# nihalsid/retrieval-fuse

Hardware: AMD Instinct MI355X
Metric: 64^3 TSDF chunks/sec (retrieve+attend+refine) (higher is better)
Workload: dtype f32

## Files before the change

retrieval-fuse_amd/csrc/build.py:

```python
import os
import subprocess
import sys
from concurrent.futures import ThreadPoolExecutor
from pathlib import Path

HERE = Path(__file__).resolve().parent
OUT = HERE.parent / 'rfuse' / 'librfuse_hip.so'
SOURCES = ['capi.hip', 'conv3d.hip', 'conv3d_mfma.hip', 'conv3d_up.hip', 'conv3d_up_split.hip', 'conv3d_split.hip', 'conv3d_split_zc.hip', 'conv3d_e2_split.hip', 'conv3d_small.hip', 'conv3d_backward.hip', 'conv3d_wgrad_split.hip', 'conv_valid_mfma.hip', 'conv_valid_split.hip', 'conv_valid_split_pg.hip', 'conv_valid_backward.hip', 'linear.hip', 'attention.hip', 'attention_fused.hip', 'retrieval.hip', 'mesh.hip', 'metrics.hip', 'mesh_metrics.hip']
FLAGS = ['--offload-arch=gfx950', '-O3', '-std=c++17', '-fPIC', '-Wall', '-Wno-unused-function']
EXTRA_FLAGS = {'attention.hip': ['-ffp-contract=off'], 'attention_fused.hip': ['-ffp-contract=off'], 'retrieval.hip': ['-ffp-contract=off'],
               'mesh_metrics.hip': ['-ffp-contract=off'],
               'conv3d_mfma.hip': ['-fno-slp-vectorize'], 'conv3d_up.hip': ['-fno-slp-vectorize']}


def _hipcc():
    return os.environ.get('HIPCC', '/opt/rocm/bin/hipcc')


def _llvm_bin():
    import shutil
    roots = [Path(os.path.realpath(_hipcc())).parents[1], Path(os.environ.get('ROCM_PATH', '/opt/rocm')), Path('/opt/rocm')]
    for r in roots:
        for sub in ('lib/llvm/bin', 'llvm/bin'):
            if (r / sub / 'llvm-objdump').exists():
# ... 33 lines not shown
        for co in cos:
            asm = subprocess.run([str(llvm_bin / 'llvm-objdump'), '-d', str(co)], check=True, capture_output=True, text=True).stdout
            bad += unsafe_packed_fp32(asm)
    if bad:
        raise RuntimeError('check_isa: %d packed-fp32 instructions with op_sel on src1/src2 (wrong results beside F16 MFMAs on gfx950), e.g.\n  %s'
                           % (len(bad), '\n  '.join(bad[:5])))
    return len(cos)


def build(force=False, verbose=False, out=None, extra_flags=(), objdir=None):
    hipcc = _hipcc()
    OUT = Path(out) if out is not None else globals()['OUT']
    objdir = Path(objdir) if objdir is not None else HERE / 'build'
    objdir.mkdir(exist_ok=True, parents=True)
    headers = [HERE / 'common.h', HERE / 'conv_box.h', HERE / 'conv_split_common.h', HERE / 'split_operand.h', HERE / 'attn_row.h', HERE / 'philox.h',
               HERE.parents[1] / 'include' / 'rfuse.h', HERE.parents[1] / 'include' / 'rfuse_eval.h']

    def compile_one(src):
        obj = objdir / (src.replace('.hip', '.o'))
        if force or _stale(obj, [HERE / src, HERE / 'build.py'] + headers):
            cmd = [hipcc] + FLAGS + list(extra_flags) + EXTRA_FLAGS.get(src, []) + ['-c', str(HERE / src), '-o', str(obj)]
            if verbose:
                print(' '.join(cmd))
            subprocess.run(cmd, check=True)
        return obj

    with ThreadPoolExecutor(max_workers=len(SOURCES)) as ex:
        objs = list(ex.map(compile_one, SOURCES))
    if force or _stale(OUT, objs):
        tmp_out = OUT.with_name(OUT.name + '.unchecked')
        cmd = [hipcc, '--offload-arch=gfx950', '-shared', '-fPIC', '-o', str(tmp_out)] + [str(o) for o in objs]
# ... 27 lines not shown
```

retrieval-fuse_amd/csrc/conv3d_split.hip:

```cpp
#include "common.h"
#include "conv_box.h"
#include "conv_split_common.h"
#include <type_traits>

bool rf_split_zc_takes(int cin, int n, int edge, int cout);
int rf_split_zc_launch(const ConvArgs& a, const SplitPreOut& po, hipStream_t stream);
bool rf_split_zcm_takes(int cin, int n, int edge, int cout);
int rf_split_zcm_launch(const ConvArgs& a, const SplitPreOut& po, bool pre, hipStream_t stream, const char* who);
int rf_split_zcm_launch_ch8_pointwise(const ConvArgs& a, const SplitPreOut& po, hipStream_t stream, const char* who);

extern "C" size_t rf_conv3_split_packed_bytes(int cout, int cin) {
    return ((size_t)((cin + 7) / 8) * 7 + 1) * (size_t)(rf_round_up(cout, 16) / 16) * 2 * 64 * 16;
}

__global__ void k_conv3_split_pack(const float* __restrict__ w, int cout, int cin, int nb_count, h8* __restrict__ wp, size_t total) {
    const size_t nreal = (size_t)((cin + 7) / 8) * 7 * nb_count * 128;
    for (size_t i = (size_t)blockIdx.x * blockDim.x + threadIdx.x; i < total; i += (size_t)gridDim.x * blockDim.x) {
        const int lane = (int)(i & 63), piece = (int)((i >> 6) & 1);
        const size_t f = i >> 7;
        const int nb = (int)(f % nb_count);
        const size_t st = f / nb_count;
        const int co = nb * 16 + (lane & 15), g = lane >> 4;
        const int s = (int)(st % 7), ca = (int)(st / 7), tap = 4 * s + g;
        h8 out;
// ... 395 lines not shown
    conv_box_epilogue<4, 4, 4, 8, 8, 4, NB, (size_t)S4_LDS_BYTES>(a, acc, reinterpret_cast<float*>(lds), tid, lane, wave, n0, 0, 0, 0, cob, lblock);
}

struct Cin1PreArgs {
    const float* src;
    const float* gamma_in;
    const float* beta_in;
    double eps_in;
    const float* wp;
    int n, cin4, cout16;
    const float* gamma;
    const float* beta;
    int cpg;
    double eps;
    unsigned char* out;
};

__global__ __launch_bounds__(512, 4) void k_conv3_cin1_presplit(Cin1PreArgs a) {
    constexpr int E = 16, H = 18, VOL = E * E * E;
    __shared__ float xs[H * H * H];
    __shared__ __attribute__((aligned(16))) float wl[27 * 8];
    __shared__ double red[8 * 16];
    __shared__ float4 nxt[8];
    const int tid = threadIdx.x, lane = tid & 63, wave = tid >> 6;
    const int nn = blockIdx.x;
    for (int i = tid; i < H * H * H; i += 512) xs[i] = 0.f;
    for (int i = tid; i < 27 * 8; i += 512) wl[i] = a.wp[(size_t)(i / 8) * a.cin4 * a.cout16 + (i % 8)];
    const float* src = a.src + (size_t)nn * VOL;
    float raw[8];
#pragma unroll
    for (int i = 0; i < 8; ++i) raw[i] = src[tid + i * 512];
    {
        double sm = 0.0, sq = 0.0;
#pragma unroll
        for (int i = 0; i < 8; ++i) { sm += (double)raw[i]; sq += (double)raw[i] * raw[i]; }
        sm = wave_sum(sm); sq = wave_sum(sq);
        if (lane == 0) { red[2 * wave] = sm; red[2 * wave + 1] = sq; }
    }
    __syncthreads();
    float4 af;
    {
        double sm = 0.0, sq = 0.0;
        for (int w = 0; w < 8; ++w) { sm += red[2 * w]; sq += red[2 * w + 1]; }
        af = rf_gn_triple(sm, sq, VOL, a.eps_in, a.gamma_in[0], a.beta_in[0]);
    }
    __syncthreads();
#pragma unroll
    for (int i = 0; i < 8; ++i) {
        const int v = tid + i * 512;
        xs[((v >> 8) + 1) * (H * H) + (((v >> 4) & 15) + 1) * H + (v & 15) + 1] = fmaf(raw[i] - af.x, af.y, af.z);
    }
    __syncthreads();
    const int x = tid & 15, y = (tid >> 4) & 15, z0 = (tid >> 8) * 8;
    typedef float f32x2 __attribute__((ext_vector_type(2)));
    f32x2 acc2[8][4];
#pragma unroll
    for (int z = 0; z < 8; ++z)
#pragma unroll
        for (int cp = 0; cp < 4; ++cp) acc2[z][cp] = (f32x2){0.f, 0.f};
#pragma unroll
    for (int dy = 0; dy < 3; ++dy)
// ... 8 lines not shown
                const float4 w1 = *reinterpret_cast<const float4*>(wl + ((dz * 3 + dy) * 3 + dx) * 8 + 4);
                const f32x2 wv[4] = {(f32x2){w0.x, w0.y}, (f32x2){w0.z, w0.w}, (f32x2){w1.x, w1.y}, (f32x2){w1.z, w1.w}};
#pragma unroll
                for (int z = 0; z < 8; ++z) {
                    const f32x2 c2 = (f32x2){col[z + dz], col[z + dz]};
#pragma unroll
                    for (int cp = 0; cp < 4; ++cp) acc2[z][cp] = __builtin_elementwise_fma(c2, wv[cp], acc2[z][cp]);
                }
            }
        }
    float act[8][8];
#pragma unroll
    for (int z = 0; z < 8; ++z)
#pragma unroll
        for (int co = 0; co < 8; ++co) act[z][co] = rf_relu(acc2[z][co >> 1][co & 1]);
    {
        double v[16];
#pragma unroll
        for (int co = 0; co < 8; ++co) {
            double sm = 0.0, sq = 0.0;
#pragma unroll
            for (int z = 0; z < 8; ++z) { const double t = (double)act[z][co]; sm += t; sq += t * t; }
            v[2 * co] = sm; v[2 * co + 1] = sq;
        }
        auto halve = [&](auto kc) {
            constexpr int K = decltype(kc)::value, C = 8 >> K;
            const bool up = (lane >> K) & 1;
#pragma unroll
            for (int i = 0; i < C; ++i) {
                const double send = up ? v[i] : v[i + C], keep = up ? v[i + C] : v[i];
                v[i] = keep + __shfl_xor(send, 1 << K, 64);
            }
        };
        halve(std::integral_constant<int, 0>{});
        halve(std::integral_constant<int, 1>{});
        halve(std::integral_constant<int, 2>{});
        halve(std::integral_constant<int, 3>{});
        v[0] += __shfl_xor(v[0], 16, 64);
        v[0] += __shfl_xor(v[0], 32, 64);
        if (lane < 16) red[wave * 16 + ((lane & 1) * 8 + ((lane >> 1) & 1) * 4 + ((lane >> 2) & 1) * 2 + ((lane >> 3) & 1))] = v[0];
    }
    __syncthreads();
    if (tid < 8) {
        const int g0 = tid / a.cpg * a.cpg;
        double sm = 0.0, sq = 0.0;
        for (int c = g0; c < g0 + a.cpg; ++c)
            for (int w = 0; w < 8; ++w) { sm += red[w * 16 + 2 * c]; sq += red[w * 16 + 2 * c + 1]; }
        nxt[tid] = rf_gn_triple(sm, sq, (double)a.cpg * VOL, a.eps, a.gamma[tid], a.beta[tid]);
    }
    __syncthreads();
    f32x2 negc[4], sc[4], sh[4];
#pragma unroll
    for (int cp = 0; cp < 4; ++cp) {
        const float4 t0 = nxt[2 * cp], t1 = nxt[2 * cp + 1];
        negc[cp] = (f32x2){-t0.x, -t1.x};
        sc[cp] = (f32x2){t0.y * SPLIT_ACT_SCALE, t1.y * SPLIT_ACT_SCALE};
        sh[cp] = (f32x2){t0.z * SPLIT_ACT_SCALE, t1.z * SPLIT_ACT_SCALE};
    }
    typedef _Float16 h2 __attribute__((ext_vector_type(2)));
    unsigned char* outp = a.out + (size_t)nn * 2 * VOL * 16;
#pragma unroll
    for (int z = 0; z < 8; ++z) {
        h8 h, l;
#pragma unroll
// ... 2 lines not shown
            f32x2 v = __builtin_elementwise_fma(relu + negc[cp], sc[cp], sh[cp]);
            v[0] = rf_clamp_f16(v[0]);
            v[1] = rf_clamp_f16(v[1]);
            const h2 hh = __builtin_convertvector(v, h2);
            const f32x2 back = __builtin_convertvector(hh, f32x2);
            const h2 ll = __builtin_convertvector((v - back) * SPLIT_LO, h2);
            h[2 * cp] = hh[0]; h[2 * cp + 1] = hh[1];
            l[2 * cp] = ll[0]; l[2 * cp + 1] = ll[1];
        }
        const size_t vox = ((size_t)(z0 + z) * E + y) * E + x;
        *reinterpret_cast<h8*>(outp + vox * 16) = h;
        *reinterpret_cast<h8*>(outp + ((size_t)VOL + vox) * 16) = l;
    }
}

extern "C" size_t rf_split_act_bytes(int n, int c, int edge) {
    return (size_t)n * (size_t)((c + 7) / 8) * 2 * (size_t)edge * edge * edge * 16;
}

extern "C" int rf_conv3d_cin1_presplit_supported(int n, int edge, int cout, int next_groups) {
    return n > 0 && edge == 16 && cout == 8 && next_groups > 0 && 8 % next_groups == 0;
}

extern "C" int rf_conv3d_cin1_presplit(const float* src, int n, int edge, const float* in_gamma, const float* in_beta, float in_eps, const float* w_packed,
                                       int cout, const float* next_gamma, const float* next_beta, int next_groups, float eps, void* out_presplit,
                                       void* stream) {
    RF_REQUIRE(rf_conv3d_cin1_presplit_supported(n, edge, cout, next_groups), RF_E_UNSUPPORTED,
               "rf_conv3d_cin1_presplit: takes 1 -> 8 channels on 16^3 samples with 1, 2, 4 or 8 groups in the consumer's GroupNorm (got n=%d edge=%d cout=%d groups=%d)",
               n, edge, cout, next_groups);
    RF_REQUIRE(src && in_gamma && in_beta && w_packed && next_gamma && next_beta && out_presplit, RF_E_INVALID, "rf_conv3d_cin1_presplit: null pointer");
    Cin1PreArgs a;
    a.src = src; a.gamma_in = in_gamma; a.beta_in = in_beta; a.eps_in = (double)in_eps; a.wp = w_packed; a.n = n; a.cin4 = 4; a.cout16 = 16;
    a.gamma = next_gamma; a.beta = next_beta; a.cpg = 8 / next_groups; a.eps = (double)eps; a.out = reinterpret_cast<unsigned char*>(out_presplit);
    hipLaunchKernelGGL(k_conv3_cin1_presplit, dim3((unsigned)n), dim3(512), 0, (hipStream_t)stream, a);
    RF_CHECK_LAUNCH("rf_conv3d_cin1_presplit");
    return RF_OK;
}

extern "C" int rf_conv3d_split_supported(int c0, int c1, int n, int edge, int cout) {
    if (edge == 4) return c1 == 0 && c0 >= 8 && c0 % 8 == 0 && n >= 1024 && cout > 0;
    if (c1 != 0 || c0 < 6 || 4 * c0 < 3 * rf_round_up(c0, 8) || n <= 0 || cout <= 0 || !rf_is_pow2(edge) || edge < 8 || edge > 128) return 0;
    const int cout16 = rf_round_up(cout, 16);
    const long long boxes = (long long)n * (edge / 8) * (edge / 8) * (edge / 8);
    if (cout16 <= 32) return rf_conv_use_big(n, edge, cout16) || boxes >= 256;
    return cout16 <= 192 && boxes * (cout16 / 16) >= 512;
}

template <int NB, int WPS, bool ONE, bool PADC = false, bool PRE = false>
static int launch_split(const ConvArgs& a, hipStream_t stream, const SplitPreOut& po = SplitPreOut{nullptr, nullptr, nullptr, 0, 0.f, nullptr, nullptr, nullptr, 0.f, 0.f}) {
    auto kern = k_conv3_split<NB, WPS, ONE, PADC, PRE>;
// ... 223 lines not shown
```

retrieval-fuse_amd/model/unet.py:

```python
import math

import torch
from torch import nn

from rfuse import ops


class GroupNormParams(nn.Module):

    def __init__(self, num_groups, num_channels, eps=1e-5):
        super().__init__()
        if num_channels < num_groups:
            num_groups = 1
        assert num_channels % num_groups == 0, \
            f'Expected number of channels in input to be divisible by num_groups. num_channels={num_channels}, num_groups={num_groups}'
        self.num_groups, self.num_channels, self.eps = num_groups, num_channels, eps
        self.weight = nn.Parameter(torch.ones(num_channels))
        self.bias = nn.Parameter(torch.zeros(num_channels))

    def extra_repr(self):
        return f'{self.num_groups}, {self.num_channels}, eps={self.eps}'


class Conv3dParams(nn.Module):
# ... 155 lines not shown
        if encoder:
            c1_in, c1_out = in_channels, max(out_channels // 2, in_channels)
            c2_in, c2_out = c1_out, out_channels
        else:
            c1_in, c1_out = in_channels, out_channels
            c2_in, c2_out = out_channels, out_channels
        self.SingleConv1 = SingleConv(c1_in, c1_out, kernel_size, order, num_groups)
        self.SingleConv2 = SingleConv(c2_in, c2_out, kernel_size, order, num_groups)

    def forward(self, x, upsampled=None, pool=None, next_block=None):
        c1, c2 = self.SingleConv1, self.SingleConv2
        if isinstance(x, ops.PreSplit):
            g2 = c2.groupnorm
            mid = ops.conv3d_split_pre_presplit(x, c1.conv.packed_split(), c1.conv.out_channels, g2.weight, g2.bias, _groups_of(g2), g2.eps)
            return ops.conv3d_split_pre_relu(mid.data, mid.channels, mid.n, mid.edge, c2.conv.packed_split(), c2.conv.out_channels, pool=pool)
        if upsampled is None and self._presplit_ok(x):
            g1, g2 = c1.groupnorm, c2.groupnorm
            n, edge, cmid, cout = x.shape[0], x.shape[2], c1.conv.out_channels, c2.conv.out_channels
            pre = ops.conv3d_cin1_presplit(x, g1.weight, g1.bias, g1.eps, c1.conv.packed(), cmid, g2.weight, g2.bias, g2.num_groups, g2.eps)
            if pool == 'only' and next_block is not None and next_block.accepts_prepooled(n, cout, edge // 2):
                ng = next_block.SingleConv1.groupnorm
                if ops.conv_split_pre_pool_presplit_supported(cmid, n, edge, cout, _groups_of(ng)):
                    _, handed = ops.conv3d_split_pre_relu_pool_presplit(pre, cmid, n, edge, c2.conv.packed_split(), cout, ng.weight, ng.bias, _groups_of(ng), ng.eps)
                    return None, handed
            return ops.conv3d_split_pre_relu(pre, cmid, n, edge, c2.conv.packed_split(), cout, pool=pool)
        if upsampled is not None and pool is None and _decoder_pair_presplit_ok(c1, c2, x, upsampled):
            return _decoder_pair_presplit(c1, c2, x, upsampled)
        if upsampled is None and x is not None and self._box_pair_presplit_ok(x):
            g1, g2 = c1.groupnorm, c2.groupnorm
            aff = ops.gn_affine(x, None, g1.weight, g1.bias, g1.num_groups, g1.eps)
            pre = ops.conv3d_split_presplit(x, aff, c1.conv.packed_split(), c1.conv.out_channels, g2.weight, g2.bias, _groups_of(g2), g2.eps)
            return ops.conv3d_split_pre_relu(pre, c1.conv.out_channels, x.shape[0], x.shape[2], c2.conv.packed_split(), c2.conv.out_channels, pool=pool)
        return c2(c1(x, upsampled), pool=pool)

    def accepts_prepooled(self, n, cin, edge):
        c1, c2 = self.SingleConv1, self.SingleConv2
        g1, g2 = c1.groupnorm, c2.groupnorm
        if torch.is_grad_enabled() and any(p.requires_grad for p in self.parameters()):
            return False
        if c1.conv.in_channels != cin:
            return False
        cmid = c1.conv.out_channels
        if not ops.conv_split_pre_presplit_supported(cin, n, edge, cmid, _groups_of(g2)) or not bool(ops._lib.load().rf_conv3d_split_pre_supported(cmid, n, edge, c2.conv.out_channels)):
            return False
        return (ops.split_range_ok(c1.conv.weight, g1.weight, g1.bias, _group_elements(g1, edge))
                and ops.split_range_ok(c2.conv.weight, g2.weight, g2.bias, _group_elements(g2, edge)))

    def _box_pair_presplit_ok(self, x):
# ... 135 lines not shown
```

retrieval-fuse_amd/rfuse/_lib.py:

```python
import ctypes
import os
import re
from pathlib import Path

import torch

_HERE = Path(__file__).resolve().parent
LIB_PATH = Path(os.environ.get('RFUSE_LIB', _HERE / 'librfuse_hip.so'))
HEADER_PATH = _HERE.parents[1] / 'include' / 'rfuse.h'
EVAL_HEADER_PATH = _HERE.parents[1] / 'include' / 'rfuse_eval.h'

_SCALARS = {'int': ctypes.c_int, 'float': ctypes.c_float, 'size_t': ctypes.c_size_t, 'int64_t': ctypes.c_int64, 'long long': ctypes.c_int64}


def parse_header(text):
    text = re.sub(r'/\*.*?\*/', ' ', text, flags=re.S)
    text = re.sub(r'^[ \t]*#.*$', ' ', text, flags=re.M)
    text = re.sub(r'extern\s+"C"\s*\{|\}', ' ', text)

    def where(chunk):
        m = re.search(r'(\w+)\s*\(', chunk)
        return '%s: %r' % (m.group(1) if m else '?', ' '.join(chunk.split()))

    *decls, rest = text.split(';')
    if rest.strip():
# ... 12 lines not shown
    table = {}
    for decl in decls:
        m = re.fullmatch(r'\s*([\w\s*]+?)\b(\w+)\s*\(([\w\s*,]*)\)\s*', decl)
        if m is None:
            raise ValueError('cannot read the declaration of %s' % where(decl))
        ret, fn, params = m.groups()
        params = [] if params.strip() == 'void' else [re.fullmatch(r'\s*(\w[\w\s*]*[\s*])(\w+)\s*', q) for q in params.split(',')]
        if None in params:
            raise ValueError('%s: every parameter needs a type and a name' % fn)
        table[fn] = (ctype(ret, fn, True), [ctype(q.group(1), fn) for q in params], [q.group(2) for q in params])
    return table


SIGNATURES = parse_header(HEADER_PATH.read_text())
EVAL_SIGNATURES = parse_header(EVAL_HEADER_PATH.read_text())


def is_status(name, table=None):
    res, _, params = (SIGNATURES if table is None else table)[name]
    return res is ctypes.c_int and params[-1:] == ['stream']


def _raise_on_status(rc, fn, args):
    if rc != 0:
        check(rc, fn.__name__)
    return rc


_lib = None
_eval = None


class _Library:

    def __init__(self, cdll, table=SIGNATURES):
        self._cdll = cdll
        self._table = table
        self._direct = {}
        for name, (res, args, _) in table.items():
            fn = getattr(cdll, name)
            fn.restype = res
            fn.argtypes = args
            if is_status(name, table):
                fn.errcheck = _raise_on_status
            self._direct[name] = fn
            setattr(self, name, fn)

    def start_profile(self, records, only=None):
        def timed(name, fn):
            def call(*args):
                e0, e1 = torch.cuda.Event(enable_timing=True), torch.cuda.Event(enable_timing=True)
                e0.record()
                rc = fn(*args)
                e1.record()
                records.append((name, tuple(a for a in args if isinstance(a, int)), e0, e1, tuple(i for i, a in enumerate(args) if a is None or (isinstance(a, ctypes.c_void_p) and not a.value))))
                return rc
            return call
        for name, (res, args, _) in self._table.items():
            if only is not None and name not in only:
                continue
            if res is ctypes.c_int and args:
                setattr(self, name, timed(name, self._direct[name]))

    def stop_profile(self):
        for name, fn in self._direct.items():
            setattr(self, name, fn)


def load():
    global _lib
    if _lib is not None:
        return _lib
    if not LIB_PATH.exists():
        raise RuntimeError(
            'librfuse_hip.so not found at %s -- build it with `python retrieval-fuse_amd/csrc/build.py` '
            '(or __graft_entry__.build()).  There is no CPU fallback for the refinement hot path.' % LIB_PATH)
    _lib = _Library(ctypes.CDLL(str(LIB_PATH)))
    return _lib


def load_eval():
    global _eval
    if _eval is None:
        _eval = _Library(load()._cdll, EVAL_SIGNATURES)
    return _eval


def check(rc, what):
    if rc != 0:
        msg = load().rf_last_error()
        raise RuntimeError('%s failed (rc=%d): %s' % (what, rc, msg.decode() if msg else ''))
```

retrieval-fuse_amd/rfuse/database.py:

```python
import torch

from . import ops


def shard_bounds(n_rows, rank, world):
    base, rem = divmod(n_rows, world)
    lo = rank * base + min(rank, rem)
    return lo, lo + base + (1 if rank < rem else 0)


def make_host_group(group=None):
    import torch.distributed as dist
    if dist.get_backend(group) == 'gloo':
        return group if group is not None else dist.group.WORLD
    ranks = dist.get_process_group_ranks(group) if group is not None else list(range(dist.get_world_size()))
    return dist.new_group(ranks=ranks, backend='gloo')


class QueryCountCheck:

    def __init__(self, host_group):
        import torch.distributed as dist
        self.host_group = host_group
        self.world = dist.get_world_size(host_group)
# ... 173 lines not shown
            half_store = vols.dtype == torch.float16 or self._fits_float16(vols)
        if half_store and vols.dtype != torch.float16:
            narrowed = torch.empty(vols.shape, dtype=torch.float16, device=self.device)
            for lo in range(0, vols.shape[0], 1024):
                piece = vols[lo:lo + 1024].to(self.device, torch.float32)
                half = piece.to(torch.float16)
                if not torch.equal(torch.nan_to_num(half.to(torch.float32), nan=0.0), torch.nan_to_num(piece, nan=0.0)) or not torch.equal(half.isnan(), piece.isnan()):
                    raise ValueError('half_store=True: the voxel store holds values float16 cannot represent (the reference\'s scenes are float16, '
                                     'dataset/scene.py:61,71); keep the float32 store for this database')
                narrowed[lo:lo + 1024] = half
            vols = narrowed
        self.half_store = bool(half_store)
        self.volumes = vols.to(self.device, torch.float16 if half_store else torch.float32).contiguous()
        self.n_scenes = self.volumes.shape[0]
        self.feature_cache = None

    @torch.no_grad()
    def build_feature_cache(self, retrieval_backbone, config, rows_per_batch=4096):
        from .configs import truncations
        d = config['dataset_train']
        _, trunc_t = truncations(config)
        n = self.n_rows
        feats = None
        for lo in range(0, n, rows_per_batch):
            hi = min(lo + rows_per_batch, n)
            m = self.meta[lo:hi]
            pad = (-m.shape[0]) % 64
            if pad:
                m = torch.cat([m, self.meta[-1:].expand(pad, 7)])
            patches = ops.gather_patches(self.volumes, m.reshape(-1, 1, 7).contiguous(), m.shape[0] // 64, 1, trunc_t, 1.0,
                                         d['target_mean'], d['target_std'], layout=1)
            f = retrieval_backbone(patches)[:hi - lo]
            if feats is None:
                feats = torch.empty((n,) + tuple(f.shape[1:]), dtype=torch.float32, device=self.device)
            feats[lo:hi] = f
        self.feature_cache = feats
        return feats

    def local_topk(self, q, k2):
        return self.backend.topk(q.contiguous(), self.emb_packed, self.hi - self.lo, self.lo, k2, **self._scan_kw)

    def local_topk_keys(self, q, k2):
        return self.backend.topk_keys(q.contiguous(), self.emb_packed, self.hi - self.lo, self.lo, k2, **self._scan_kw)

    def search(self, q, k2):
        if self.world == 1 and not self.force_collectives:
            return self.local_topk(q, k2)
        if self.count_check is None:
            self.count_check = QueryCountCheck(make_host_group(self.group))
        return sharded_search(q, lambda qa: self.local_topk_keys(qa, k2), self.backend.merge_keys, k2, self.group, self.collective_events,
                              self.count_check)

    def check(self):
# ... 7 lines not shown
```

retrieval-fuse_amd/rfuse/engine.py:

```python
import contextlib
import functools
import io

import torch

import model as rf_model
from . import ops
from .configs import truncations


def _on_engine_device(method):
    @functools.wraps(method)
    def scoped(self, *args, **kwargs):
        if self.device.index == torch.cuda.current_device():
            return method(self, *args, **kwargs)
        with torch.cuda.device(self.device):
            return method(self, *args, **kwargs)
    return scoped


class RefinementEngine:
    def __init__(self, config, device='cuda:0', database=None, quiet=True):
        self.config = config
        self.device = torch.device(device)
# ... 10 lines not shown
            self.fenc_input, self.fenc_target = rf_model.get_retrieval_networks(config['retrieval_model'])
        for m in list(self.modules().values()) + ([self.fenc_target] if self.fenc_target is not None else []):
            m.to(self.device).eval()
        self.database = database
        self._side_streams = {}
        self.serial = False
        self.front_at = 'start'

    def modules(self):
        return {'unet_backbone': self.unet_backbone, 'decoder': self.decoder, 'retrieval_backbone': self.retrieval_backbone,
                'patched_attention_block': self.patched_attention_block, 'fenc_input': self.fenc_input}

    def load_state_dicts(self, sds):
        for name, sd in sds.items():
            self.modules()[name].load_state_dict(sd)

    def load_checkpoints(self, refinement_ckpt=None, retrieval_ckpt=None, trust_pickle=False):
        from . import checkpoint
        loaded = []
        if refinement_ckpt is not None:
            loaded += checkpoint.load_prefixed(self.modules(), refinement_ckpt, checkpoint.REFINEMENT_PREFIXES, self.device, trust_pickle)
        if retrieval_ckpt is not None:
            loaded += checkpoint.load_prefixed({'fenc_input': self.fenc_input, 'fenc_target': self.fenc_target}, retrieval_ckpt,
                                               checkpoint.RETRIEVAL_PREFIXES, self.device, trust_pickle)
        return loaded

    @_on_engine_device
    @torch.no_grad()
    def embed_queries(self, input_raw):
        g, d = self.config['query_geometry'], self.config['dataset_train']
        pad = 0.0 if self.config['task'] == 'surface_reconstruction' else self.input_trunc
        z = ops.embed_windows(self.fenc_input, input_raw, g['patch_size_input'], g['patch_context_input'], pad, d['input_mean'], d['input_std'])
        return ops.l2_normalize_rows_(z.reshape(z.shape[0], z.shape[1]))

    @_on_engine_device
    @torch.no_grad()
    def retrieve(self, input_raw, query_scene=None, patch_mask=None, q=None):
        d = self.config['dataset_train']
        if q is None:
            q = self.embed_queries(input_raw)
        keep = patch_mask.reshape(-1).contiguous() if patch_mask is not None else None
        meta, _, _ = self.database.retrieve(q, self.K, query_scene, keep)
        patches = ops.gather_patches(self.database.volumes, meta, input_raw.shape[0], self.K, self.target_trunc, 1.0,
                                     d['target_mean'], d['target_std'], layout=1)
        return patches, meta

    @_on_engine_device
    @torch.no_grad()
    def normalise_input(self, input_raw):
        d = self.config['dataset_train']
        s = input_raw.shape[-1]
        return ops.query_windows(input_raw, s, 0, 0.0, d['input_mean'], d['input_std']).reshape(input_raw.shape[0], 1, s, s, s)

    def _fork_backbone(self, x_in):
        main = torch.cuda.current_stream(self.device)
        if self.serial:
            return self.unet_backbone(x_in), main
        side = self._side_streams.get(main.cuda_stream)
        if side is None:
            side = self._side_streams[main.cuda_stream] = torch.cuda.Stream(self.device)
# ... 22 lines not shown

    @_on_engine_device
    @torch.no_grad()
    def refine(self, input_raw, query_scene=None, gumbel_noise=None, use_feature_cache=False, patch_mask=None):
        x_back, side = self._fork_backbone(self.normalise_input(input_raw))
        q = self.embed_queries(input_raw)
        if use_feature_cache:
            if self.database.feature_cache is None:
                raise RuntimeError('use_feature_cache=True needs database.build_feature_cache(retrieval_backbone, config) first')
            b = input_raw.shape[0]
            keep = patch_mask.reshape(-1).contiguous() if patch_mask is not None else None
            _, _, idx = self.database.retrieve(q, self.K, query_scene, keep)
            order = idx.reshape(b, 64, self.K).permute(0, 2, 1).reshape(-1).contiguous()
            feats = ops.gather_rows(self.database.feature_cache, order)
        else:
            patches, _ = self.retrieve(input_raw, query_scene, patch_mask, q=q)
            feats = self.retrieval_backbone(patches)
        torch.cuda.current_stream(self.device).wait_stream(side)
        df = self._attend_and_decode(x_back, feats, gumbel_noise)
        self._check_database()
        return df

    def _check_database(self):
        if self.database is not None and not torch.cuda.is_current_stream_capturing():
            self.database.check()

    def refine_stream(self, batches, query_scenes=None, patch_masks=None):
        pending = None
        main = None
        state = {}

        def issue_front(raw, qs, pm, with_backbone=True):
            front = self._side_streams.get(('front', main.cuda_stream))
            if front is None:
                front = self._side_streams[('front', main.cuda_stream)] = torch.cuda.Stream(self.device)
            ready = torch.cuda.Event()
            ready.record(main)
            front.wait_event(ready)
            with torch.cuda.stream(front):
                raw.record_stream(front)
                x_in = self.normalise_input(raw)
                if with_backbone:
                    x_back, side = self._fork_backbone(x_in)
                patches, _ = self.retrieve(raw, qs, pm)
                if with_backbone:
                    front.wait_stream(side)
                done = torch.cuda.Event()
                done.record(front)
            return (patches, x_back, done) if with_backbone else (patches, x_in, done)

        front_at = self.front_at
        if front_at not in ('start', 'decoders', 'unet_decoders'):
            raise ValueError("RefinementEngine.front_at must be 'start', 'decoders' or 'unet_decoders', got %r" % (front_at,))
        for i, raw in enumerate(batches):
            qs = query_scenes[i] if query_scenes is not None else None
            pm = patch_masks[i] if patch_masks is not None else None
            with torch.cuda.device(self.device), torch.no_grad():
                if main is None:
                    main = torch.cuda.current_stream(self.device)
# ... 49 lines not shown
```

retrieval-fuse_amd/rfuse/ops.py:

```python
import ctypes
import functools
import sys
import weakref

import torch

from . import _lib

ACT_NONE, ACT_RELU, ACT_LEAKY = 0, 1, 2
ATTN_SOFTMAX, ATTN_GUMBEL_HARD = 0, 1


def _req(t, name, dtype=torch.float32):
    if not isinstance(t, torch.Tensor):
        raise TypeError('%s: expected a torch.Tensor' % name)
    if not t.is_cuda:
        raise RuntimeError('%s: the refinement hot path runs on the GPU only (got a %s tensor); there is no CPU fallback' % (name, t.device))
    if t.dtype != dtype:
        raise TypeError('%s: expected %s, got %s' % (name, dtype, t.dtype))
    if not t.is_contiguous():
        raise ValueError('%s: tensor must be contiguous' % name)
    return t


# ... 344 lines not shown
    n, edge = x.shape[0], x.shape[2]
    lib = _lib.load()
    return bool(lib.rf_conv3d_cin1_presplit_supported(n, edge, cout, next_groups)) and bool(lib.rf_conv3d_split_pre_supported(cout, n, edge, next_cout))


def conv3d_cin1_presplit(x, in_gamma, in_beta, in_eps, w_packed, cout, next_gamma, next_beta, next_groups, eps):
    _req(x, 'x')
    n, edge = x.shape[0], x.shape[2]
    lib = _lib.load()
    out = torch.empty(lib.rf_split_act_bytes(n, cout, edge), dtype=torch.uint8, device=x.device)
    lib.rf_conv3d_cin1_presplit(_p(x), n, edge, _p(in_gamma.detach()), _p(in_beta.detach()), in_eps, _p(w_packed), cout, _p(next_gamma.detach()),
                                _p(next_beta.detach()), next_groups, eps, _p(out), _stream())
    return out


def conv_split_pointwise_supported(x, cout):
    return CONV_ARITH == 'split' and x is not None and bool(_lib.load().rf_conv3d_split_pointwise_supported(x.shape[1], x.shape[0], x.shape[2], cout))


def conv3d_split_pointwise_tanh(x, gn_affine_t, w_split_packed, cout, pw_w, pw_b, post_add=0.0, post_mul=1.0):
    _req(x, 'x')
    n, cin, edge = x.shape[0], x.shape[1], x.shape[2]
    if pw_w.shape[0] != 1:
        raise NotImplementedError('conv3d_split_pointwise_tanh: one output channel (Conv3d(nf,1,1), model/refinement.py:54)')
    out = torch.empty((n, 1, edge, edge, edge), dtype=torch.float32, device=x.device)
    _lib.load().rf_conv3d_split_k3_gn_relu_pointwise_tanh(_p(x), cin, n, edge, _p(gn_affine_t), _p(w_split_packed), cout, _p(pw_w.detach()), _p(pw_b.detach()),
                                                          post_add, post_mul, _p(out), _stream())
    return out


# ... 731 lines not shown
```

Baseline: 5073.

## Feed level-0 cin1 conv directly from the database store with cached GroupNorm sums

The first presplit conv now reads retrieved patches straight from the database volumes using the retrieval meta, applying truncation and normalisation in the kernel. This removes the separate gather_patches materialisation and its global write and re-read. It also adds per-database-row tables of the input and first-layer GroupNorm sums, built once and invalidated when weights change, so the block-wide reductions are skipped at run time. The cost is extra code paths, a one-off table build that cannot run during graph capture, and double-precision table memory per database row.

After: 5084, median of 6. Within noise of the previous version (+0.2%).

```diff
diff --git a/include/rfuse_store.h b/include/rfuse_store.h
--- /dev/null
+++ b/include/rfuse_store.h
@@ -0,0 +1,23 @@
+#ifndef RFUSE_STORE_H
+#define RFUSE_STORE_H
+
+#include <stdint.h>
+#include <stddef.h>
+
+#ifdef __cplusplus
+extern "C" {
+#endif
+
+int rf_conv3d_cin1_presplit_store(const void* db_volumes, int store_f16, int64_t n_scenes, const int32_t* meta, int chunks, int K, float trunc_fill,
+                                  float trunc_ratio, float mean, float stddev, const int64_t* rows, int64_t n_rows, const void* in_sums,
+                                  const void* out_sums, const float* in_gamma, const float* in_beta, float in_eps, const float* w_packed, int cout,
+                                  const float* next_gamma, const float* next_beta, int next_groups, float eps, void* out_presplit, void* stream);
+int rf_level0_sums_build(const void* db_volumes, int store_f16, int64_t n_scenes, const int32_t* db_meta, int64_t n_rows, float trunc_fill,
+                         float trunc_ratio, float mean, float stddev, const float* in_gamma, const float* in_beta, float in_eps,
+                         const float* w_packed, int next_groups, void* in_sums, void* out_sums, void* stream);
+
+#ifdef __cplusplus
+}
+#endif
+
+#endif
diff --git a/retrieval-fuse_amd/csrc/build.py b/retrieval-fuse_amd/csrc/build.py
--- a/retrieval-fuse_amd/csrc/build.py
+++ b/retrieval-fuse_amd/csrc/build.py
@@ -71,7 +71,7 @@
     objdir = Path(objdir) if objdir is not None else HERE / 'build'
     objdir.mkdir(exist_ok=True, parents=True)
     headers = [HERE / 'common.h', HERE / 'conv_box.h', HERE / 'conv_split_common.h', HERE / 'split_operand.h', HERE / 'attn_row.h', HERE / 'philox.h',
-               HERE.parents[1] / 'include' / 'rfuse.h', HERE.parents[1] / 'include' / 'rfuse_eval.h']
+               HERE.parents[1] / 'include' / 'rfuse.h', HERE.parents[1] / 'include' / 'rfuse_eval.h', HERE.parents[1] / 'include' / 'rfuse_store.h']
 
     def compile_one(src):
         obj = objdir / (src.replace('.hip', '.o'))
diff --git a/retrieval-fuse_amd/csrc/conv3d_split.hip b/retrieval-fuse_amd/csrc/conv3d_split.hip
--- a/retrieval-fuse_amd/csrc/conv3d_split.hip
+++ b/retrieval-fuse_amd/csrc/conv3d_split.hip
@@ -2,6 +2,7 @@
 #include "conv_box.h"
 #include "conv_split_common.h"
 #include <type_traits>
+#include "../../include/rfuse_store.h"
 
 bool rf_split_zc_takes(int cin, int n, int edge, int cout);
 int rf_split_zc_launch(const ConvArgs& a, const SplitPreOut& po, hipStream_t stream);
@@ -433,37 +434,94 @@
     int cpg;
     double eps;
     unsigned char* out;
+    const void* store;
+    long long n_scenes;
+    const int* meta;
+    int K;
+    float trunc_fill, ratio, mean, stddev;
+    const long long* rows;
+    long long n_rows;
+    const double2* in_sums;
+    const double2* out_sums;
+    double2* in_sums_w;
+    double2* out_sums_w;
 };
 
-__global__ __launch_bounds__(512, 4) void k_conv3_cin1_presplit(Cin1PreArgs a) {
+template <int SRC, bool BUILD>
+__device__ __forceinline__ void cin1_presplit_body(const Cin1PreArgs& a) {
     constexpr int E = 16, H = 18, VOL = E * E * E;
     __shared__ float xs[H * H * H];
     __shared__ __attribute__((aligned(16))) float wl[27 * 8];
     __shared__ double red[8 * 16];
     __shared__ float4 nxt[8];
+    __shared__ float4 afs;
     const int tid = threadIdx.x, lane = tid & 63, wave = tid >> 6;
     const int nn = blockIdx.x;
+    const bool conv = !BUILD || a.out_sums_w != nullptr;
     for (int i = tid; i < H * H * H; i += 512) xs[i] = 0.f;
-    for (int i = tid; i < 27 * 8; i += 512) wl[i] = a.wp[(size_t)(i / 8) * a.cin4 * a.cout16 + (i % 8)];
-    const float* src = a.src + (size_t)nn * VOL;
+    if (conv)
+        for (int i = tid; i < 27 * 8; i += 512) wl[i] = a.wp[(size_t)(i / 8) * a.cin4 * a.cout16 + (i % 8)];
     float raw[8];
-#pragma unroll
-    for (int i = 0; i < 8; ++i) raw[i] = src[tid + i * 512];
-    {
+    long long entry = BUILD ? (long long)nn : a.n_rows;
+    if constexpr (SRC == 0) {
+        const float* src = a.src + (size_t)nn * VOL;
+#pragma unroll
+        for (int i = 0; i < 8; ++i) raw[i] = src[tid + i * 512];
+    } else {
+        typedef typename std::conditional<SRC == 1, _Float16, float>::type T;
+        const int* m;
+        bool have = true;
+        if constexpr (BUILD) {
+            m = a.meta + (size_t)nn * 7;
+            have = nn < a.n_rows;
+        } else {
+            const int slot = nn & 63, k = (nn >> 6) % a.K, chunk = (nn >> 6) / a.K;
+            const size_t mi = ((size_t)chunk * 64 + slot) * a.K + k;
+            m = a.meta + mi * 7;
+            if (a.rows) {
+                const long long r = a.rows[mi];
+                if (r >= 0 && r < a.n_rows) entry = r;
+            }
+        }
+        int scene = -1, x0 = 0, y0 = 0, z0 = 0;
+        if (have) { scene = m[0]; x0 = m[1]; y0 = m[3]; z0 = m[5]; }
+        have = scene >= 0 && scene < a.n_scenes;
+        const T* src = reinterpret_cast<const T*>(a.store) + (size_t)(have ? scene : 0) * 64 * 64 * 64;
+#pragma unroll
+        for (int i = 0; i < 8; ++i) {
+            const int v = tid + i * 512;
+            float t = a.trunc_fill;
+            if (have) t = (float)src[((size_t)(x0 + (v >> 8)) * 64 + (y0 + ((v >> 4) & 15))) * 64 + (z0 + (v & 15))];
+            t = __fmul_rn(t, a.ratio);
+            asm volatile("" : "+v"(t));
+            raw[i] = __fdiv_rn(__fsub_rn(t, a.mean), a.stddev);
+        }
+    }
+    const bool tab_in = SRC != 0 && !BUILD && a.in_sums != nullptr, tab_out = SRC != 0 && !BUILD && a.out_sums != nullptr;
+    if (!tab_in) {
         double sm = 0.0, sq = 0.0;
 #pragma unroll
         for (int i = 0; i < 8; ++i) { sm += (double)raw[i]; sq += (double)raw[i] * raw[i]; }
         sm = wave_sum(sm); sq = wave_sum(sq);
         if (lane == 0) { red[2 * wave] = sm; red[2 * wave + 1] = sq; }
-    }
+        __syncthreads();
+    }
+    if (tid == 0) {
+        double sm = 0.0, sq = 0.0;
+        if (tab_in) {
+            const double2 t = a.in_sums[entry];
+            sm = t.x; sq = t.y;
+        } else {
+            for (int w = 0; w < 8; ++w) { sm += red[2 * w]; sq += red[2 * w + 1]; }
+        }
+        if constexpr (BUILD) {
+            if (a.in_sums_w) a.in_sums_w[nn] = make_double2(sm, sq);
+        }
+        if (conv) afs = rf_gn_triple(sm, sq, VOL, a.eps_in, a.gamma_in[0], a.beta_in[0]);
+    }
+    if (!conv) return;
     __syncthreads();
-    float4 af;
-    {
-        double sm = 0.0, sq = 0.0;
-        for (int w = 0; w < 8; ++w) { sm += red[2 * w]; sq += red[2 * w + 1]; }
-        af = rf_gn_triple(sm, sq, VOL, a.eps_in, a.gamma_in[0], a.beta_in[0]);
-    }
-    __syncthreads();
+    const float4 af = afs;
 #pragma unroll
     for (int i = 0; i < 8; ++i) {
         const int v = tid + i * 512;
@@ -502,7 +560,7 @@
     for (int z = 0; z < 8; ++z)
 #pragma unroll
         for (int co = 0; co < 8; ++co) act[z][co] = rf_relu(acc2[z][co >> 1][co & 1]);
-    {
+    if (!tab_out) {
         double v[16];
 #pragma unroll
         for (int co = 0; co < 8; ++co) {
@@ -527,15 +585,25 @@
         v[0] += __shfl_xor(v[0], 16, 64);
         v[0] += __shfl_xor(v[0], 32, 64);
         if (lane < 16) red[wave * 16 + ((lane & 1) * 8 + ((lane >> 1) & 1) * 4 + ((lane >> 2) & 1) * 2 + ((lane >> 3) & 1))] = v[0];
-    }
-    __syncthreads();
+        __syncthreads();
+    }
     if (tid < 8) {
-        const int g0 = tid / a.cpg * a.cpg;
         double sm = 0.0, sq = 0.0;
-        for (int c = g0; c < g0 + a.cpg; ++c)
-            for (int w = 0; w < 8; ++w) { sm += red[w * 16 + 2 * c]; sq += red[w * 16 + 2 * c + 1]; }
-        nxt[tid] = rf_gn_triple(sm, sq, (double)a.cpg * VOL, a.eps, a.gamma[tid], a.beta[tid]);
-    }
+        if (tab_out) {
+            const double2 t = a.out_sums[entry * 8 + tid];
+            sm = t.x; sq = t.y;
+        } else {
+            const int g0 = tid / a.cpg * a.cpg;
+            for (int c = g0; c < g0 + a.cpg; ++c)
+                for (int w = 0; w < 8; ++w) { sm += red[w * 16 + 2 * c]; sq += red[w * 16 + 2 * c + 1]; }
+        }
+        if constexpr (BUILD) {
+            a.out_sums_w[(size_t)nn * 8 + tid] = make_double2(sm, sq);
+        } else {
+            nxt[tid] = rf_gn_triple(sm, sq, (double)a.cpg * VOL, a.eps, a.gamma[tid], a.beta[tid]);
+        }
+    }
+    if constexpr (BUILD) return;
     __syncthreads();
     f32x2 negc[4], sc[4], sh[4];
 #pragma unroll
@@ -568,6 +636,10 @@
     }
 }
 
+__global__ __launch_bounds__(512, 4) void k_conv3_cin1_presplit(Cin1PreArgs a) { cin1_presplit_body<0, false>(a); }
+template <int SRC, bool BUILD>
+__global__ __launch_bounds__(512, 4) void k_conv3_cin1_store(Cin1PreArgs a) { cin1_presplit_body<SRC, BUILD>(a); }
+
 extern "C" size_t rf_split_act_bytes(int n, int c, int edge) {
     return (size_t)n * (size_t)((c + 7) / 8) * 2 * (size_t)edge * edge * edge * 16;
 }
@@ -583,11 +655,55 @@
                "rf_conv3d_cin1_presplit: takes 1 -> 8 channels on 16^3 samples with 1, 2, 4 or 8 groups in the consumer's GroupNorm (got n=%d edge=%d cout=%d groups=%d)",
                n, edge, cout, next_groups);
     RF_REQUIRE(src && in_gamma && in_beta && w_packed && next_gamma && next_beta && out_presplit, RF_E_INVALID, "rf_conv3d_cin1_presplit: null pointer");
-    Cin1PreArgs a;
+    Cin1PreArgs a = {};
     a.src = src; a.gamma_in = in_gamma; a.beta_in = in_beta; a.eps_in = (double)in_eps; a.wp = w_packed; a.n = n; a.cin4 = 4; a.cout16 = 16;
     a.gamma = next_gamma; a.beta = next_beta; a.cpg = 8 / next_groups; a.eps = (double)eps; a.out = reinterpret_cast<unsigned char*>(out_presplit);
     hipLaunchKernelGGL(k_conv3_cin1_presplit, dim3((unsigned)n), dim3(512), 0, (hipStream_t)stream, a);
     RF_CHECK_LAUNCH("rf_conv3d_cin1_presplit");
+    return RF_OK;
+}
+
+extern "C" int rf_conv3d_cin1_presplit_store(const void* db_volumes, int store_f16, int64_t n_scenes, const int32_t* meta, int chunks, int K, float trunc_fill,
+                                             float trunc_ratio, float mean, float stddev, const int64_t* rows, int64_t n_rows, const void* in_sums,
+                                             const void* out_sums, const float* in_gamma, const float* in_beta, float in_eps, const float* w_packed, int cout,
+                                             const float* next_gamma, const float* next_beta, int next_groups, float eps, void* out_presplit, void* stream) {
+    RF_REQUIRE(chunks > 0 && K > 0 && (long long)chunks * K * 64 <= 0x7fffffffLL && n_scenes > 0, RF_E_INVALID,
+               "rf_conv3d_cin1_presplit_store: bad arguments (chunks=%d K=%d)", chunks, K);
+    const int n = chunks * K * 64;
+    RF_REQUIRE(rf_conv3d_cin1_presplit_supported(n, 16, cout, next_groups), RF_E_UNSUPPORTED,
+               "rf_conv3d_cin1_presplit_store: takes 1 -> 8 channels with 1, 2, 4 or 8 groups in the consumer's GroupNorm (got cout=%d groups=%d)", cout, next_groups);
+    RF_REQUIRE(db_volumes && meta && in_gamma && in_beta && w_packed && next_gamma && next_beta && out_presplit, RF_E_INVALID,
+               "rf_conv3d_cin1_presplit_store: null pointer");
+    RF_REQUIRE((!in_sums && !out_sums) || (rows && n_rows >= 0), RF_E_INVALID, "rf_conv3d_cin1_presplit_store: a table needs the row ids");
+    Cin1PreArgs a = {};
+    a.gamma_in = in_gamma; a.beta_in = in_beta; a.eps_in = (double)in_eps; a.wp = w_packed; a.n = n; a.cin4 = 4; a.cout16 = 16;
+    a.gamma = next_gamma; a.beta = next_beta; a.cpg = 8 / next_groups; a.eps = (double)eps; a.out = reinterpret_cast<unsigned char*>(out_presplit);
+    a.store = db_volumes; a.n_scenes = (long long)n_scenes; a.meta = meta; a.K = K;
+    a.trunc_fill = trunc_fill; a.ratio = trunc_ratio; a.mean = mean; a.stddev = stddev;
+    a.rows = reinterpret_cast<const long long*>(rows); a.n_rows = (long long)n_rows;
+    a.in_sums = reinterpret_cast<const double2*>(in_sums); a.out_sums = reinterpret_cast<const double2*>(out_sums);
+    if (store_f16) hipLaunchKernelGGL((k_conv3_cin1_store<1, false>), dim3((unsigned)n), dim3(512), 0, (hipStream_t)stream, a);
+    else hipLaunchKernelGGL((k_conv3_cin1_store<2, false>), dim3((unsigned)n), dim3(512), 0, (hipStream_t)stream, a);
+    RF_CHECK_LAUNCH("rf_conv3d_cin1_presplit_store");
+    return RF_OK;
+}
+
+extern "C" int rf_level0_sums_build(const void* db_volumes, int store_f16, int64_t n_scenes, const int32_t* db_meta, int64_t n_rows, float trunc_fill,
+                                    float trunc_ratio, float mean, float stddev, const float* in_gamma, const float* in_beta, float in_eps,
+                                    const float* w_packed, int next_groups, void* in_sums, void* out_sums, void* stream) {
+    RF_REQUIRE(db_volumes && db_meta && n_rows >= 0 && n_rows < 0x7fffffffLL && n_scenes > 0 && (in_sums || out_sums), RF_E_INVALID,
+               "rf_level0_sums_build: bad arguments");
+    RF_REQUIRE(!out_sums || (in_gamma && in_beta && w_packed && next_groups > 0 && 8 % next_groups == 0), RF_E_INVALID,
+               "rf_level0_sums_build: out_sums needs the first layer's parameters and 1, 2, 4 or 8 groups (got %d)", next_groups);
+    Cin1PreArgs a = {};
+    a.gamma_in = in_gamma; a.beta_in = in_beta; a.eps_in = (double)in_eps; a.wp = w_packed; a.n = (int)n_rows + 1; a.cin4 = 4; a.cout16 = 16;
+    a.cpg = out_sums ? 8 / next_groups : 8;
+    a.store = db_volumes; a.n_scenes = (long long)n_scenes; a.meta = db_meta; a.K = 1;
+    a.trunc_fill = trunc_fill; a.ratio = trunc_ratio; a.mean = mean; a.stddev = stddev; a.n_rows = (long long)n_rows;
+    a.in_sums_w = reinterpret_cast<double2*>(in_sums); a.out_sums_w = reinterpret_cast<double2*>(out_sums);
+    if (store_f16) hipLaunchKernelGGL((k_conv3_cin1_store<1, true>), dim3((unsigned)n_rows + 1), dim3(512), 0, (hipStream_t)stream, a);
+    else hipLaunchKernelGGL((k_conv3_cin1_store<2, true>), dim3((unsigned)n_rows + 1), dim3(512), 0, (hipStream_t)stream, a);
+    RF_CHECK_LAUNCH("rf_level0_sums_build");
     return RF_OK;
 }
 
diff --git a/retrieval-fuse_amd/model/unet.py b/retrieval-fuse_amd/model/unet.py
--- a/retrieval-fuse_amd/model/unet.py
+++ b/retrieval-fuse_amd/model/unet.py
@@ -193,10 +193,16 @@
             g2 = c2.groupnorm
             mid = ops.conv3d_split_pre_presplit(x, c1.conv.packed_split(), c1.conv.out_channels, g2.weight, g2.bias, _groups_of(g2), g2.eps)
             return ops.conv3d_split_pre_relu(mid.data, mid.channels, mid.n, mid.edge, c2.conv.packed_split(), c2.conv.out_channels, pool=pool)
-        if upsampled is None and self._presplit_ok(x):
+        level0 = upsampled is None and self._presplit_ok(x)
+        if isinstance(x, ops.StorePatches) and not level0:
+            x = x.materialise()
+        if level0:
             g1, g2 = c1.groupnorm, c2.groupnorm
             n, edge, cmid, cout = x.shape[0], x.shape[2], c1.conv.out_channels, c2.conv.out_channels
-            pre = ops.conv3d_cin1_presplit(x, g1.weight, g1.bias, g1.eps, c1.conv.packed(), cmid, g2.weight, g2.bias, g2.num_groups, g2.eps)
+            if isinstance(x, ops.StorePatches):
+                pre = self._cin1_presplit_store(x)
+            else:
+                pre = ops.conv3d_cin1_presplit(x, g1.weight, g1.bias, g1.eps, c1.conv.packed(), cmid, g2.weight, g2.bias, g2.num_groups, g2.eps)
             if pool == 'only' and next_block is not None and next_block.accepts_prepooled(n, cout, edge // 2):
                 ng = next_block.SingleConv1.groupnorm
                 if ops.conv_split_pre_pool_presplit_supported(cmid, n, edge, cout, _groups_of(ng)):
@@ -211,6 +217,22 @@
             pre = ops.conv3d_split_presplit(x, aff, c1.conv.packed_split(), c1.conv.out_channels, g2.weight, g2.bias, _groups_of(g2), g2.eps)
             return ops.conv3d_split_pre_relu(pre, c1.conv.out_channels, x.shape[0], x.shape[2], c2.conv.packed_split(), c2.conv.out_channels, pool=pool)
         return c2(c1(x, upsampled), pool=pool)
+
+    def _cin1_presplit_store(self, h):
+        c1, c2 = self.SingleConv1, self.SingleConv2
+        g1, g2 = c1.groupnorm, c2.groupnorm
+        w = c1.conv.packed()
+        in_sums = out_sums = None
+        if h.tables is not None and h.rows is not None and (ops.USE_IN_SUMS or ops.USE_OUT_SUMS):
+            first = key = None
+            if ops.USE_OUT_SUMS:
+                first = (g1.weight, g1.bias, g1.eps, w, g2.num_groups)
+                key = tuple((t.data_ptr(), t._version) for t in (g1.weight, g1.bias, c1.conv.weight)) + (g1.eps, g2.num_groups)
+            in_sums, out_sums = h.tables.level0_sums(h.constants(), key, first)
+            if not ops.USE_IN_SUMS:
+                in_sums = None
+        return ops.conv3d_cin1_presplit_store(h, g1.weight, g1.bias, g1.eps, w, c1.conv.out_channels, g2.weight, g2.bias, g2.num_groups, g2.eps,
+                                              in_sums=in_sums, out_sums=out_sums)
 
     def accepts_prepooled(self, n, cin, edge):
         c1, c2 = self.SingleConv1, self.SingleConv2
diff --git a/retrieval-fuse_amd/rfuse/_lib.py b/retrieval-fuse_amd/rfuse/_lib.py
--- a/retrieval-fuse_amd/rfuse/_lib.py
+++ b/retrieval-fuse_amd/rfuse/_lib.py
@@ -9,6 +9,7 @@
 LIB_PATH = Path(os.environ.get('RFUSE_LIB', _HERE / 'librfuse_hip.so'))
 HEADER_PATH = _HERE.parents[1] / 'include' / 'rfuse.h'
 EVAL_HEADER_PATH = _HERE.parents[1] / 'include' / 'rfuse_eval.h'
+STORE_HEADER_PATH = _HERE.parents[1] / 'include' / 'rfuse_store.h'
 
 _SCALARS = {'int': ctypes.c_int, 'float': ctypes.c_float, 'size_t': ctypes.c_size_t, 'int64_t': ctypes.c_int64, 'long long': ctypes.c_int64}
 
@@ -51,6 +52,7 @@
 
 SIGNATURES = parse_header(HEADER_PATH.read_text())
 EVAL_SIGNATURES = parse_header(EVAL_HEADER_PATH.read_text())
+STORE_SIGNATURES = parse_header(STORE_HEADER_PATH.read_text())
 
 
 def is_status(name, table=None):
@@ -66,6 +68,7 @@
 
 _lib = None
 _eval = None
+_store = None
 
 
 class _Library:
@@ -74,6 +77,7 @@
         self._cdll = cdll
         self._table = table
         self._direct = {}
+        self._also = []
         for name, (res, args, _) in table.items():
             fn = getattr(cdll, name)
             fn.restype = res
@@ -98,10 +102,14 @@
                 continue
             if res is ctypes.c_int and args:
                 setattr(self, name, timed(name, self._direct[name]))
+        for other in self._also:
+            other.start_profile(records, only)
 
     def stop_profile(self):
         for name, fn in self._direct.items():
             setattr(self, name, fn)
+        for other in self._also:
+            other.stop_profile()
 
 
 def load():
@@ -123,6 +131,15 @@
     return _eval
 
 
+def load_store():
+    global _store
+    if _store is None:
+        main = load()
+        _store = _Library(main._cdll, STORE_SIGNATURES)
+        main._also.append(_store)
+    return _store
+
+
 def check(rc, what):
     if rc != 0:
         msg = load().rf_last_error()
diff --git a/retrieval-fuse_amd/rfuse/database.py b/retrieval-fuse_amd/rfuse/database.py
--- a/retrieval-fuse_amd/rfuse/database.py
+++ b/retrieval-fuse_amd/rfuse/database.py
@@ -211,6 +211,8 @@
         self.volumes = vols.to(self.device, torch.float16 if half_store else torch.float32).contiguous()
         self.n_scenes = self.volumes.shape[0]
         self.feature_cache = None
+        self._level0_in = None
+        self._level0_out = None
 
     @torch.no_grad()
     def build_feature_cache(self, retrieval_backbone, config, rows_per_batch=4096):
@@ -234,6 +236,32 @@
         self.feature_cache = feats
         return feats
 
+    def level0_sums(self, constants, first_key=None, first=None):
+        made = False
+        if self._level0_in is None or self._level0_in[0] != constants:
+            self._check_not_capturing()
+            self._level0_in = (constants, ops.level0_sums_build(self.volumes, self.meta, constants)[0])
+            self._level0_out = None
+            made = True
+        out_sums = None
+        if first is not None:
+            if self._level0_out is None or self._level0_out[0] != first_key:
+                self._check_not_capturing()
+                self._level0_out = (first_key, ops.level0_sums_build(self.volumes, self.meta, constants, first, want_in=False)[1])
+                made = True
+            out_sums = self._level0_out[1]
+        if made:
+            torch.cuda.current_stream(self.device).synchronize()
+        return self._level0_in[1], out_sums
+
+    def drop_level0_out_sums(self):
+        self._level0_out = None
+
+    @staticmethod
+    def _check_not_capturing():
+        if torch.cuda.is_current_stream_capturing():
+            raise RuntimeError('the level-0 sum tables would be built inside a graph capture: run one step before capturing (RefinementEngine.capture_graph does)')
+
     def local_topk(self, q, k2):
         return self.backend.topk(q.contiguous(), self.emb_packed, self.hi - self.lo, self.lo, k2, **self._scan_kw)
 
diff --git a/retrieval-fuse_amd/rfuse/engine.py b/retrieval-fuse_amd/rfuse/engine.py
--- a/retrieval-fuse_amd/rfuse/engine.py
+++ b/retrieval-fuse_amd/rfuse/engine.py
@@ -48,6 +48,11 @@
     def load_state_dicts(self, sds):
         for name, sd in sds.items():
             self.modules()[name].load_state_dict(sd)
+        self._weights_replaced()
+
+    def _weights_replaced(self):
+        if self.database is not None:
+            self.database.drop_level0_out_sums()
 
     def load_checkpoints(self, refinement_ckpt=None, retrieval_ckpt=None, trust_pickle=False):
         from . import checkpoint
@@ -57,6 +62,7 @@
         if retrieval_ckpt is not None:
             loaded += checkpoint.load_prefixed({'fenc_input': self.fenc_input, 'fenc_target': self.fenc_target}, retrieval_ckpt,
                                                checkpoint.RETRIEVAL_PREFIXES, self.device, trust_pickle)
+        self._weights_replaced()
         return loaded
 
     @_on_engine_device
@@ -78,6 +84,19 @@
         patches = ops.gather_patches(self.database.volumes, meta, input_raw.shape[0], self.K, self.target_trunc, 1.0,
                                      d['target_mean'], d['target_std'], layout=1)
         return patches, meta
+
+    @_on_engine_device
+    @torch.no_grad()
+    def retrieve_store(self, input_raw, query_scene=None, patch_mask=None, q=None):
+        if not ops.USE_STORE_FED:
+            return self.retrieve(input_raw, query_scene, patch_mask, q=q)[0]
+        d = self.config['dataset_train']
+        if q is None:
+            q = self.embed_queries(input_raw)
+        keep = patch_mask.reshape(-1).contiguous() if patch_mask is not None else None
+        meta, _, rows = self.database.retrieve(q, self.K, query_scene, keep)
+        return ops.StorePatches(self.database.volumes, meta, rows, input_raw.shape[0], self.K, self.target_trunc, 1.0, d['target_mean'], d['target_std'],
+                                tables=self.database)
 
     @_on_engine_device
     @torch.no_grad()
@@ -130,7 +149,7 @@
             order = idx.reshape(b, 64, self.K).permute(0, 2, 1).reshape(-1).contiguous()
             feats = ops.gather_rows(self.database.feature_cache, order)
         else:
-            patches, _ = self.retrieve(input_raw, query_scene, patch_mask, q=q)
+            patches = self.retrieve_store(input_raw, query_scene, patch_mask, q=q)
             feats = self.retrieval_backbone(patches)
         torch.cuda.current_stream(self.device).wait_stream(side)
         df = self._attend_and_decode(x_back, feats, gumbel_noise)
@@ -158,7 +177,7 @@
                 x_in = self.normalise_input(raw)
                 if with_backbone:
                     x_back, side = self._fork_backbone(x_in)
-                patches, _ = self.retrieve(raw, qs, pm)
+                patches = self.retrieve_store(raw, qs, pm)
                 if with_backbone:
                     front.wait_stream(side)
                 done = torch.cuda.Event()
diff --git a/retrieval-fuse_amd/rfuse/ops.py b/retrieval-fuse_amd/rfuse/ops.py
--- a/retrieval-fuse_amd/rfuse/ops.py
+++ b/retrieval-fuse_amd/rfuse/ops.py
@@ -382,6 +382,60 @@
     return out
 
 
+USE_STORE_FED = True
+USE_IN_SUMS = True
+USE_OUT_SUMS = True
+
+
+class StorePatches:
+    requires_grad = False
+
+    def __init__(self, volumes, meta, rows, chunks, K, trunc_fill, trunc_ratio, mean, std, tables=None):
+        self.volumes, self.meta, self.rows, self.chunks, self.K = volumes, meta, rows, chunks, K
+        self.trunc_fill, self.trunc_ratio, self.mean, self.std = float(trunc_fill), float(trunc_ratio), float(mean), float(std)
+        self.tables = tables
+        self.shape = (chunks * K * 64, 1, 16, 16, 16)
+        self.device = volumes.device
+
+    def constants(self):
+        return self.trunc_fill, self.trunc_ratio, self.mean, self.std
+
+    def materialise(self):
+        return gather_patches(self.volumes, self.meta, self.chunks, self.K, *self.constants(), layout=1)
+
+    def record_stream(self, stream):
+        self.meta.record_stream(stream)
+        if self.rows is not None:
+            self.rows.record_stream(stream)
+
+
+def level0_sums_build(volumes, db_meta, constants, first=None, want_in=True):
+    half = volumes.dtype == torch.float16
+    _req(volumes, 'volumes', torch.float16 if half else torch.float32), _req(db_meta, 'db_meta', torch.int32)
+    r, dev = db_meta.shape[0], volumes.device
+    in_sums = torch.empty((r + 1, 2), dtype=torch.float64, device=dev) if want_in else None
+    out_sums = torch.empty((r + 1, 8, 2), dtype=torch.float64, device=dev) if first is not None else None
+    g, b, eps, w, groups = first if first is not None else (None, None, 0.0, None, 1)
+    _lib.load_store().rf_level0_sums_build(_p(volumes), int(half), volumes.shape[0], _p(db_meta), r, *constants, _p(g.detach()) if g is not None else None,
+                                     _p(b.detach()) if b is not None else None, eps, _p(w), groups, _p(in_sums), _p(out_sums), _stream())
+    return in_sums, out_sums
+
+
+def conv3d_cin1_presplit_store(h, in_gamma, in_beta, in_eps, w_packed, cout, next_gamma, next_beta, next_groups, eps, in_sums=None, out_sums=None):
+    half = h.volumes.dtype == torch.float16
+    _req(h.volumes, 'volumes', torch.float16 if half else torch.float32), _req(h.meta, 'meta', torch.int32)
+    n_rows, rows = 0, None
+    if in_sums is not None or out_sums is not None:
+        rows = h.rows
+        _req(rows, 'rows', torch.int64)
+        n_rows = (in_sums if in_sums is not None else out_sums).shape[0] - 1
+    out = torch.empty(_lib.load().rf_split_act_bytes(h.shape[0], cout, 16), dtype=torch.uint8, device=h.device)
+    _lib.load_store().rf_conv3d_cin1_presplit_store(_p(h.volumes), int(half), h.volumes.shape[0], _p(h.meta), h.chunks, h.K, *h.constants(), _p(rows),
+                                      n_rows, _p(in_sums), _p(out_sums), _p(in_gamma.detach()), _p(in_beta.detach()), in_eps, _p(w_packed), cout,
+                                      _p(next_gamma.detach()), _p(next_beta.detach()), next_groups, eps, _p(out), _stream())
+    return out
+
+
 def conv_split_pointwise_supported(x, cout):
     return CONV_ARITH == 'split' and x is not None and bool(_lib.load().rf_conv3d_split_pointwise_supported(x.shape[1], x.shape[0], x.shape[2], cout))
 
```
